# gaurav00700/Selfsupervised-NVSF

Hardware: AMD Instinct MI355X
Metric: rendered rays/sec (LiDAR+cam) (higher is better)
Workload: dtype f16; 1 GPU; C2: KITTI-360 seq-1908-shaped frame per GPU, uniform sampling, static hash field; num_rays=4096, num_rays_lidar=4096, num_steps=768, hash_grid=L16 F2 T2^19 base16 max2048, sigma_mlp=32-64-16, heads=lidar 2x(87-64-64-1), rgb 31-64-64-3, parallelism=frame-sharded x1, no collective

## Files before the change

selfsupervised-nvsf_amd/csrc/common.h:

```cpp
#pragma once
#include <hip/hip_runtime.h>
#include <stdint.h>

#define NVSF_API extern "C" __attribute__((visibility("default")))

enum : int {
    NVSF_OK = 0,
    NVSF_ERR_INVALID_ARG = -1,
    NVSF_ERR_UNSUPPORTED = -2,
};

constexpr int kWave = 64;

static inline int nvsf_launch_status() {
    hipError_t e = hipGetLastError();
    return e == hipSuccess ? NVSF_OK : (int)e;
}

static inline unsigned cdiv(unsigned long long a, unsigned b) { return (unsigned)((a + b - 1) / b); }

enum NvsfVariantKey : int {
    kVarMarch = 0,
    kVarPlanesFwd,
    kVarPlanesBwd,
    kVarHashgridFwd,
    kVarHashgridBwd,
    kVarHash4dBwd,
    kVarSlicePlan,
    kVarRenderTail,
    kVarMarchSkew,
    kVarMlpBwd,
    kVarLevelKinds,
    kVarCount
};
int nvsf_variant(int key);
int nvsf_cu_count();

__device__ __forceinline__ int lane_id() { return (int)(threadIdx.x & 63); }

template <typename T>
__device__ __forceinline__ T wave_sum(T v) {
#pragma unroll
    for (int o = 32; o > 0; o >>= 1) v += __shfl_xor(v, o, 64);
    return v;
}

__device__ __forceinline__ float wave_scan_add(float v) {
    const int l = lane_id();
#pragma unroll
    for (int o = 1; o < 64; o <<= 1) {
        float u = __shfl_up(v, o, 64);
        if (l >= o) v += u;
    }
    return v;
}
__device__ __forceinline__ float wave_scan_mul(float v) {
    const int l = lane_id();
#pragma unroll
    for (int o = 1; o < 64; o <<= 1) {
        float u = __shfl_up(v, o, 64);
        if (l >= o) v *= u;
    }
    return v;
}
__device__ __forceinline__ uint32_t wave_scan_add_u32(uint32_t v) {
    const int l = lane_id();
#pragma unroll
    for (int o = 1; o < 64; o <<= 1) {
        uint32_t u = __shfl_up(v, o, 64);
        if (l >= o) v += u;
    }
    return v;
}

__device__ __forceinline__ uint32_t wave_scan_max_u32(uint32_t v) {
#define NVSF_DPP_MAX(ctrl, row_mask)                                                                                        \
    {                                                                                                                      \
        const uint32_t u = (uint32_t)__builtin_amdgcn_update_dpp(0, (int)v, ctrl, row_mask, 0xF, false);                   \
        v = u > v ? u : v;                                                                                                 \
    }
    NVSF_DPP_MAX(0x111, 0xF)
    NVSF_DPP_MAX(0x112, 0xF)
    NVSF_DPP_MAX(0x114, 0xF)
    NVSF_DPP_MAX(0x118, 0xF)
    NVSF_DPP_MAX(0x142, 0xA)
    NVSF_DPP_MAX(0x143, 0xC)
#undef NVSF_DPP_MAX
    return v;
}
```

selfsupervised-nvsf_amd/csrc/fused_field.hip:

```cpp
#include "hashgrid_device.h"
#include "mlp_device.h"
#include "encodings_device.h"
#include "march_device.h"
#pragma clang diagnostic ignored "-Wpass-failed"
#include <stdlib.h>

namespace {
constexpr int kBlock = 256;
constexpr int kWavesPerBlock = kBlock / kWave;

struct RayBatch {
    const float* rays_o;
    const float* rays_d;
    const float* nears;
    const float* fars;
    const float* lin;
    const float* noise;
    float lo[3], hi[3];
    float inv_extent;
    float bound;
    uint32_t N, T;
};

template <int F>
// ... 18 lines not shown
        const unsigned long long s = in_range ? s_raw : total - 1;
        const uint32_t n = (uint32_t)(s / rb.T), i = (uint32_t)(s - (unsigned long long)n * rb.T);
        const float near = rb.nears[n], range = rb.fars[n] - near;
        float z = near + range * rb.lin[i];
        if (rb.noise) z = z + (rb.noise[s] - 0.5f) * (range / (float)rb.T);
        float x[3];
#pragma unroll
        for (int k = 0; k < 3; ++k) {
            float p = rb.rays_o[3 * (size_t)n + k] + rb.rays_d[3 * (size_t)n + k] * z;
            p = fminf(fmaxf(p, rb.lo[k]), rb.hi[k]);
            x[k] = (p + rb.bound) * rb.inv_extent;
        }
        half8_t xf;
#pragma unroll
        for (int q = 0; q < kLevelsPerGroup; ++q) {
            const int l = g * kLevelsPerGroup + q;
            float acc[F];
            encode_level<3, F>(x, table, meta.scale[l], meta.res[l], meta.offset[l], meta.offset[l + 1] - meta.offset[l], acc);
#pragma unroll
            for (int f = 0; f < F; ++f) xf[q * F + f] = (_Float16)acc[f];
        }
        float4_t acc1[kHidTiles];
#pragma unroll
        for (int t = 0; t < kHidTiles; ++t) {
            const float4_t zero = {0, 0, 0, 0};
            acc1[t] = mfma16(w0[t], xf, zero);
        }
        half8_t h[kHidSteps];
        pack_hidden(acc1, h);
        const float4_t o = wout.apply(h);
        if (in_range) {
            half4_t ov;
            ov[0] = (_Float16)o[0]; ov[1] = (_Float16)o[1]; ov[2] = (_Float16)o[2]; ov[3] = (_Float16)o[3];
            if (g == 3) {
                z_vals[s] = z;
                sigmas[s] = expf(o[3]);
                ov[3] = (_Float16)1.0f;
            }
            *reinterpret_cast<half4_t*>(geo + s * 16 + 4 * g) = ov;
        }
    }
}

template <int F>
struct LaneLevels {
    static constexpr int Q = 8 / F;
    float scale[Q];
    uint32_t res[Q], res2[Q], boff[Q], rows[Q];
};

__device__ __forceinline__ void fma_entry(float w, uint32_t raw, float& a0, float& a1) {
    asm("v_fma_mix_f32 %0, %1, %2, %0 op_sel_hi:[0,1,0]" : "+v"(a0) : "v"(w), "v"(raw));
    asm("v_fma_mix_f32 %0, %1, %2, %0 op_sel:[0,1,0] op_sel_hi:[0,1,0]" : "+v"(a1) : "v"(w), "v"(raw));
}

template <int F>
__device__ __forceinline__ uint32_t gather_raw(__amdgpu_buffer_rsrc_t rsrc, uint32_t byte_off);
template <>
__device__ __forceinline__ uint32_t gather_raw<2>(__amdgpu_buffer_rsrc_t rsrc, uint32_t byte_off) {
    return __builtin_amdgcn_raw_buffer_load_b32(rsrc, byte_off, 0, 0);
}
typedef uint32_t entry4_t __attribute__((ext_vector_type(2)));
template <int F> struct EntryOf { typedef uint32_t type; };
template <> struct EntryOf<4> { typedef entry4_t type; };
template <>
__device__ __forceinline__ uint32_t gather_raw<4>(__amdgpu_buffer_rsrc_t, uint32_t) = delete;
__device__ __forceinline__ entry4_t gather_raw4(__amdgpu_buffer_rsrc_t rsrc, uint32_t byte_off) {
    return __builtin_amdgcn_raw_buffer_load_b64(rsrc, byte_off, 0, 0);
}

template <int F>
struct DensityCtx {
    static constexpr int Q = 8 / F;
    LaneLevels<F> lv;
    half8_t w0[kHidTiles];
    OutLayerW wout;
    __amdgpu_buffer_rsrc_t rsrc;
    uint32_t first_hashed;
    int g;
    const uint4* lds_lv;
};

constexpr uint32_t kFirstHashedC2 = 5;
template <int F, int QG, bool LDS_LV = false, int FH = -1>
__device__ __forceinline__ half8_t density_encode(const DensityCtx<F>& cx, const float (&x)[3]) {
    constexpr int Q = 8 / F;
    LaneLevels<F> lv_local;
    if constexpr (LDS_LV) {
        uint32_t again = 0;
        asm volatile("" : "+v"(again));
#pragma unroll
        for (int q = 0; q < Q; ++q) {
            const uint4 v = cx.lds_lv[4 * q + again];
            lv_local.scale[q] = __builtin_bit_cast(float, v.x);
            lv_local.res[q] = v.y;
            lv_local.res2[q] = v.y * v.y;
            lv_local.boff[q] = v.z;
            lv_local.rows[q] = v.w;
        }
    }
    const LaneLevels<F>& lv = LDS_LV ? lv_local : cx.lv;
    const uint32_t first_hashed = FH >= 0 ? (uint32_t)FH : cx.first_hashed;
    const int g = cx.g;
    half8_t xf;
#pragma unroll
    for (int q0 = 0; q0 < Q; q0 += QG) {
    float frac[Q][3];
    typename EntryOf<F>::type raw[Q][8];
#pragma unroll
    for (int q = q0; q < q0 + QG; ++q) {
        uint32_t c[3];
#pragma unroll
        for (int d = 0; d < 3; ++d) {
            const float pos = fmaf(lv.scale[q], x[d], 0.5f);
            const float fl = floorf(pos);
            frac[q][d] = pos - fl;
            c[d] = (uint32_t)(int32_t)fl;
        }
        uint32_t idx[8];
        const bool all_dense = (uint32_t)(4 * q + 3) < first_hashed, all_hashed = (uint32_t)(4 * q) >= first_hashed;
        if (all_dense || !all_hashed) {
            const uint32_t b00 = c[0] + c[1] * lv.res[q] + c[2] * lv.res2[q];
            const uint32_t b10 = b00 + lv.res[q], b01 = b00 + lv.res2[q], b11 = b10 + lv.res2[q];
            const uint32_t base[4] = {b00, b10, b01, b11};
#pragma unroll
            for (int k = 0; k < 8; ++k) {
                uint32_t v = base[k >> 1] + (uint32_t)(k & 1);
                v = v >= lv.rows[q] ? v - lv.rows[q] : v;
                idx[k] = v;
            }
        }
        if (all_hashed || !all_dense) {
            const uint32_t hy0 = c[1] * 2654435761u, hy1 = hy0 + 2654435761u;
            const uint32_t hz0 = c[2] * 805459861u, hz1 = hz0 + 805459861u;
            const uint32_t yz[4] = {hy0 ^ hz0, hy1 ^ hz0, hy0 ^ hz1, hy1 ^ hz1};
            const uint32_t mask = lv.rows[q] - 1u;
            const bool lane_hashed = (uint32_t)(4 * q + g) >= first_hashed;
#pragma unroll
            for (int k = 0; k < 8; ++k) {
                const uint32_t v = ((c[0] + (uint32_t)(k & 1)) ^ yz[k >> 1]) & mask;
                idx[k] = (all_hashed || lane_hashed) ? v : idx[k];
            }
        }
#pragma unroll
        for (int k = 0; k < 8; ++k) {
            if constexpr (F == 2) raw[q][k] = gather_raw<2>(cx.rsrc, lv.boff[q] + idx[k] * (uint32_t)(F * sizeof(_Float16)));
            else raw[q][k] = gather_raw4(cx.rsrc, lv.boff[q] + idx[k] * (uint32_t)(F * sizeof(_Float16)));
        }
    }
#pragma unroll
    for (int q = q0; q < q0 + QG; ++q) {
        const float fx = frac[q][0], fy = frac[q][1], fz = frac[q][2];
        const float wx[2] = {1.0f - fx, fx}, wy[2] = {1.0f - fy, fy}, wz[2] = {1.0f - fz, fz};
        if constexpr (F == 2) {
            float a0 = 0.0f, a1 = 0.0f;
#pragma unroll
            for (int k = 0; k < 8; ++k) {
                const float w = (wx[k & 1] * wy[(k >> 1) & 1]) * wz[k >> 2];
                fma_entry(w, raw[q][k], a0, a1);
            }
            xf[q * F] = (_Float16)a0;
            xf[q * F + 1] = (_Float16)a1;
        } else {
            float a0 = 0.0f, a1 = 0.0f, a2 = 0.0f, a3 = 0.0f;
#pragma unroll
            for (int k = 0; k < 8; ++k) {
                const float w = (wx[k & 1] * wy[(k >> 1) & 1]) * wz[k >> 2];
                fma_entry(w, raw[q][k][0], a0, a1);
                fma_entry(w, raw[q][k][1], a2, a3);
            }
            xf[q * F] = (_Float16)a0;
            xf[q * F + 1] = (_Float16)a1;
            xf[q * F + 2] = (_Float16)a2;
            xf[q * F + 3] = (_Float16)a3;
        }
    }
    }
    return xf;
}

template <int F, int QG>
__device__ __forceinline__ float4_t density_eval(const DensityCtx<F>& cx, const float (&x)[3]) {
    const half8_t xf = density_encode<F, QG>(cx, x);
    float4_t acc1[kHidTiles];
#pragma unroll
    for (int t = 0; t < kHidTiles; ++t) {
        const float4_t zero = {0, 0, 0, 0};
        acc1[t] = mfma16(cx.w0[t], xf, zero);
    }
    half8_t h[kHidSteps];
    pack_hidden(acc1, h);
    return cx.wout.apply(h);
}

struct TrainOut {
    float* x01;
    _Float16* feat;
    float* h32;
    uint32_t* tile;
};

__device__ __forceinline__ void store_h32(float* __restrict__ h32, unsigned long long s, int lane, int g, float o0, float o1, float o2, float o3, bool ok) {
    const int from = (lane + 48) & 63;
    const float prev = __int_as_float(__builtin_amdgcn_ds_bpermute(from << 2, __float_as_int(o3)));
    if (ok) *reinterpret_cast<float4*>(h32 + s * 16 + 4 * g) = make_float4(prev, o0, o1, o2);
}

constexpr int kTrPitch = 20;
constexpr int kTrWords = 16 * kTrPitch;
__device__ __forceinline__ void store_feat_row(_Float16* __restrict__ feat, unsigned long long s, int lane, int g, const uint4& p, bool ok,
                                               uint32_t* tile) {
    uint32_t* row = tile + (lane & 15) * kTrPitch;
    row[g] = p.x; row[4 + g] = p.y; row[8 + g] = p.z; row[12 + g] = p.w;
    const uint4 mine = *reinterpret_cast<const uint4*>(row + 4 * g);
    if (ok) *reinterpret_cast<uint4*>(feat + s * 32 + 8 * g) = mine;
}

__device__ __forceinline__ void store_feat_row_swap(_Float16* __restrict__ feat, unsigned long long s, int g, const uint4& p, bool ok) {
    const auto a = __builtin_amdgcn_permlane16_swap(p.x, p.y, false, false);
    const auto b = __builtin_amdgcn_permlane16_swap(p.z, p.w, false, false);
    const auto lo = __builtin_amdgcn_permlane32_swap(a[0], b[0], false, false);
    const auto hi = __builtin_amdgcn_permlane32_swap(a[1], b[1], false, false);
    if (ok) *reinterpret_cast<uint4*>(feat + s * 32 + 8 * g) = make_uint4(lo[0], hi[0], lo[1], hi[1]);
}

template <int F, int QG, bool TRAIN = false>
__device__ __forceinline__ void density_tile(const DensityCtx<F>& cx, const float (&x)[3], float z, unsigned long long s, bool in_range,
                                             float* __restrict__ z_vals, float* __restrict__ sigmas, _Float16* __restrict__ geo,
                                             const TrainOut* tr = nullptr) {
    const int g = cx.g;
    float4_t o;
    if constexpr (TRAIN) {
        const half8_t xf = density_encode<F, QG>(cx, x);
        float4_t acc1[kHidTiles];
#pragma unroll
        for (int t = 0; t < kHidTiles; ++t) {
            const float4_t zero = {0, 0, 0, 0};
            acc1[t] = mfma16(cx.w0[t], xf, zero);
        }
        half8_t h[kHidSteps];
        pack_hidden(acc1, h);
        o = cx.wout.apply(h);
        const int lane = lane_id();
        store_feat_row(tr->feat, s, lane, g, __builtin_bit_cast(uint4, xf), in_range, tr->tile);
        store_h32(tr->h32, s, lane, g, o[0], o[1], o[2], o[3], in_range);
        if (in_range && g == 0) { tr->x01[3 * s] = x[0]; tr->x01[3 * s + 1] = x[1]; tr->x01[3 * s + 2] = x[2]; }
    } else {
        o = density_eval<F, QG>(cx, x);
    }
    if (in_range) {
        half4_t ov;
        ov[0] = (_Float16)o[0]; ov[1] = (_Float16)o[1]; ov[2] = (_Float16)o[2]; ov[3] = (_Float16)o[3];
        if (g == 3) {
            z_vals[s] = z;
            sigmas[s] = expf(o[3]);
            ov[3] = (_Float16)1.0f;
        }
        *reinterpret_cast<half4_t*>(geo + s * 16 + 4 * g) = ov;
    }
// ... 917 lines not shown
        }
        const float sigma = expf(o[3]) * density_scale;
        const uint32_t p0 = pack_h2(o[0], o[1]), p1 = pack_h2(o[2], g == 3 ? 1.0f : o[3]);
        typedef uint32_t u4_t __attribute__((ext_vector_type(4)));
        u4_t gv;
        gv[0] = (uint32_t)__shfl((int)p0, src_a);
        gv[1] = (uint32_t)__shfl((int)p1, src_a);
        gv[2] = (uint32_t)__shfl((int)p0, src_b);
        gv[3] = (uint32_t)__shfl((int)p1, src_b);
        const half8_t x_last = takes_geo ? __builtin_bit_cast(half8_t, gv) : xf[IN_STEPS - 1];
        float c[3] = {0.0f, 0.0f, 0.0f};
        const float4_t oa = head(0, x_last);
        if constexpr (LIDAR) {
            const float4_t ob = head(1, x_last);
            c[0] = sigmoid_f32(oa[0]);
            c[1] = sigmoid_f32(ob[0]);
        } else {
            c[0] = sigmoid_f32(oa[0]); c[1] = sigmoid_f32(oa[1]); c[2] = sigmoid_f32(oa[2]);
        }
#pragma unroll
        for (int i = 0; i < 16; ++i) {
            if ((uint32_t)i < cnt && alive) {
                const float s_i = readlane_f32(sigma, 48 + i);
                const float dt_i = readlane_f32(sdt, i), d1_i = readlane_f32(sd1, i);
                const float alpha = 1.0f - expf(-s_i * dt_i);
                const float T = 1.0f - ws;
                const float w = alpha * T;
                ws += w;
                t_comp += d1_i;
                dep += w * t_comp;
#pragma unroll
                for (int k = 0; k < 3; ++k) col[k] += w * readlane_f32(c[k], i);
                if (T < T_thresh) alive = false;
            }
        }
        total += cnt;
        if (cnt < 16u) alive = false;
    }
    if (lane == 0) {
        weights_sum[n] = ws;
        depth[n] = dep;
        if constexpr (LIDAR) {
            image[2 * (size_t)n] = col[0];
            image[2 * (size_t)n + 1] = col[1];
        } else {
            const float rest = 1.0f - ws;
            image[3 * (size_t)n] = col[0] + rest * bg0;
            image[3 * (size_t)n + 1] = col[1] + rest * bg1;
            image[3 * (size_t)n + 2] = col[2] + rest * bg2;
        }
    }
}

template <int N>
__device__ __forceinline__ float row_shr(float old, float v) {
    static_assert(N >= 1 && N <= 15, "row_shr:1..15");
    return __builtin_bit_cast(float, __builtin_amdgcn_update_dpp(__builtin_bit_cast(int, old), __builtin_bit_cast(int, v), 0x110 + N, 0xF, 0xF, false));
}

__device__ __forceinline__ float row_shl1(float old, float v) {
    return __builtin_bit_cast(float, __builtin_amdgcn_update_dpp(__builtin_bit_cast(int, old), __builtin_bit_cast(int, v), 0x101, 0xF, 0xF, false));
}

__device__ __forceinline__ float row_first(float v) {
    return __builtin_bit_cast(float, __builtin_amdgcn_update_dpp(0, __builtin_bit_cast(int, v), 0x150, 0xF, 0xF, false));
}

__device__ __forceinline__ float row16_scan_mul(float v) {
    v *= row_shr<1>(1.0f, v);
    v *= row_shr<2>(1.0f, v);
    v *= row_shr<4>(1.0f, v);
    v *= row_shr<8>(1.0f, v);
    return v;
}

struct RenderTrainOut {
    float* x01;
    _Float16* feat;
    _Float16* geo;
    float* sigma;
    float* rgb;
};

template <bool LIDAR, bool FROM_FEATURES, bool TRAIN = false, int FH = -1>
__global__ __launch_bounds__(kBlock) __attribute__((amdgpu_waves_per_eu(4, 4))) void k_render_uniform(
    RayBatch rb, const _Float16* __restrict__ table, uint32_t table_bytes, GridMeta meta, uint32_t first_hashed,
    const uint2* __restrict__ feat, const _Float16* __restrict__ w_sigma, const _Float16* __restrict__ w_a, const _Float16* __restrict__ w_b,
    float k_scale, float w_thresh, float bg0, float bg1, float bg2, int use_bg, float* __restrict__ z_vals, float* __restrict__ weights,
    float* __restrict__ weights_sum, float* __restrict__ depth, float* __restrict__ image, RenderTrainOut rt = RenderTrainOut()) {
    using FR = OccFrags<LIDAR>;
    constexpr int F = 2;
    constexpr int IN_STEPS = FR::IN_STEPS;
    constexpr int C = LIDAR ? 2 : 3;
    __shared__ uint4 s_lv[kMaxLevels];
    __shared__ half8_t s_frag[FR::kCount * kWave];
    __shared__ float4_t s_pre[kWavesPerBlock * FR::kPre];
    if (threadIdx.x < kMaxLevels) {
        const uint32_t l = threadIdx.x;
        s_lv[l] = make_uint4(__builtin_bit_cast(uint32_t, meta.scale[l]), meta.res[l], meta.offset[l] * (uint32_t)(F * sizeof(_Float16)),
                             meta.offset[l + 1] - meta.offset[l]);
    }
    const int lane = lane_id(), g = lane >> 4, c = lane & 15;
    for (int f = (int)(threadIdx.x >> 6); f < FR::kCount; f += kWavesPerBlock) s_frag[f * kWave + lane] = occ_fragment<LIDAR>(f, lane, w_sigma, w_a, w_b);
    __syncthreads();
    const uint32_t n = __builtin_amdgcn_readfirstlane(blockIdx.x * kWavesPerBlock + (threadIdx.x >> 6));
    if (n >= rb.N) return;
    const half8_t* frag = s_frag + lane;
    const uint32_t T = rb.T;
    const size_t M = (size_t)rb.N * T;

    DensityCtx<F> cx;
    if constexpr (!FROM_FEATURES) {
        cx.g = g;
        cx.first_hashed = first_hashed;
        cx.lds_lv = s_lv + g;
        cx.rsrc = __builtin_amdgcn_make_buffer_rsrc(const_cast<_Float16*>(table), 0, (int)table_bytes, 0x00020000);
    }
    const float rd0 = rb.rays_d[3 * (size_t)n], rd1 = rb.rays_d[3 * (size_t)n + 1], rd2 = rb.rays_d[3 * (size_t)n + 2];
    const float d0 = (rd0 + 1.0f) / 2.0f, d1 = (rd1 + 1.0f) / 2.0f, d2 = (rd2 + 1.0f) / 2.0f;
    half8_t xf[IN_STEPS];
    if constexpr (!LIDAR) {
        float sh[16];
        sh4_basis(d0, d1, d2, sh);
#pragma unroll
        for (int j = 0; j < 8; ++j) xf[0][j] = (_Float16)(g == 0 ? sh[j] : sh[8 + j]);
    } else {
#pragma unroll
        for (int s = 0; s < 3; ++s)
#pragma unroll
            for (int j = 0; j < 8; j += 2) {
                const int k = 32 * s + 8 * g + j;
                float sn = 1.0f, cs = 1.0f;
                if (k < 72) {
                    const int i = k / 24, f = (k - 24 * i) >> 1;
                    freq_pair(i == 0 ? d0 : (i == 1 ? d1 : d2), f, sn, cs);
                }
                xf[s][j] = (_Float16)sn;
                xf[s][j + 1] = (_Float16)cs;
            }
    }
    const bool takes_geo = LIDAR ? (g == 1 || g == 2) : (g >= 2);
    const int src_a = (c + 16 * (LIDAR ? 2 * (g - 1) : 2 * (g - 2))) & 63, src_b = (src_a + 16) & 63;
    float4_t* pre = s_pre + (threadIdx.x >> 6) * FR::kPre;
    ray_head_constants<LIDAR>(xf, w_a, w_b, lane, pre);
    auto head = [&](int hd, const half8_t& x_last) {
        const int base = FR::kHead + hd * FR::kPerHead;
        float4_t acc[kHidTiles];
#pragma unroll
        for (int t = 0; t < kHidTiles; ++t) {
            float4_t c = {0, 0, 0, 0};
            if constexpr (IN_STEPS > 1) c = pre[(hd * 4 + t) * 4 + g];
            acc[t] = mfma16(frag[(base + t) * kWave], x_last, c);
        }
        half8_t h[kHidSteps];
        pack_hidden(acc, h);
#pragma unroll
        for (int t = 0; t < kHidTiles; ++t) {
            float4_t c = {0, 0, 0, 0};
#pragma unroll
            for (int s = 0; s < kHidSteps; ++s) c = mfma16(frag[(base + 4 + 2 * t + s) * kWave], h[s], c);
            acc[t] = c;
        }
        pack_hidden(acc, h);
        float4_t c = {0, 0, 0, 0};
#pragma unroll
        for (int s = 0; s < kHidSteps; ++s) c = mfma16(frag[(base + 4 + 8 + s) * kWave], h[s], c);
        return c;
    };

    const float near = rb.nears[n], range = rb.fars[n] - near;
    const float sample_dist = range / (float)T;
    const float ox = rb.rays_o[3 * (size_t)n], oy = rb.rays_o[3 * (size_t)n + 1], oz = rb.rays_o[3 * (size_t)n + 2];
    const size_t row0 = (size_t)n * T;
    float carry = 1.0f, ws = 0.0f, dp = 0.0f, img[C];
#pragma unroll
    for (int k = 0; k < C; ++k) img[k] = 0.0f;
    float lin_cur = 0.0f, lin_nxt = 0.0f, nz_cur = 0.5f, nz_nxt = 0.5f;
    auto request = [&](uint32_t i0) {
        const uint32_t i = i0 + (uint32_t)c;
        const uint32_t ic = i < T ? i : T - 1u, in = ic + 1u < T ? ic + 1u : ic;
        lin_cur = rb.lin[ic];
        lin_nxt = rb.lin[in];
        if (rb.noise) {
            nz_cur = rb.noise[row0 + ic];
            nz_nxt = rb.noise[row0 + in];
        }
    };
    if constexpr (!FROM_FEATURES) request(0u);
    for (uint32_t i0 = 0; i0 < T; i0 += 16) {
        const uint32_t i = i0 + (uint32_t)c;
        const bool valid = i < T;
        const uint32_t ic = valid ? i : T - 1u;
        const size_t s = row0 + ic;
        float z, z_next;
        half8_t feat8;
        if constexpr (FROM_FEATURES) {
            z = z_vals[s];
            z_next = ic + 1u < T ? z_vals[s + 1] : z;
            const uint2 p0 = feat[(size_t)(2 * g) * M + s], p1 = feat[(size_t)(2 * g + 1) * M + s];
            typedef uint32_t u4_t __attribute__((ext_vector_type(4)));
            const u4_t packed = {p0.x, p1.x, p1.y, p0.y};
            feat8 = __builtin_bit_cast(half8_t, packed);
        } else {
            z = near + range * lin_cur;
            z_next = near + range * lin_nxt;
            if (rb.noise) {
                z = z + (nz_cur - 0.5f) * sample_dist;
                z_next = z_next + (nz_nxt - 0.5f) * sample_dist;
            }
            if (i0 + 16u < T) request(i0 + 16u);
            float x[3];
            x[0] = (fminf(fmaxf(ox + rd0 * z, rb.lo[0]), rb.hi[0]) + rb.bound) * rb.inv_extent;
            x[1] = (fminf(fmaxf(oy + rd1 * z, rb.lo[1]), rb.hi[1]) + rb.bound) * rb.inv_extent;
            x[2] = (fminf(fmaxf(oz + rd2 * z, rb.lo[2]), rb.hi[2]) + rb.bound) * rb.inv_extent;
            feat8 = density_encode<F, 4, true, FH>(cx, x);
            if constexpr (TRAIN) {
                if (g == 0 && valid) { rt.x01[3 * s] = x[0]; rt.x01[3 * s + 1] = x[1]; rt.x01[3 * s + 2] = x[2]; }
            }
        }
        if constexpr (TRAIN) store_feat_row_swap(rt.feat, s, g, __builtin_bit_cast(uint4, feat8), valid);
        float4_t o;
        {
            float4_t acc1[kHidTiles];
#pragma unroll
            for (int tt = 0; tt < kHidTiles; ++tt) acc1[tt] = mfma16(frag[(FR::kSigma + tt) * kWave], feat8, float4_t{0, 0, 0, 0});
            half8_t h[kHidSteps];
            pack_hidden(acc1, h);
            float4_t a = {0, 0, 0, 0};
#pragma unroll
            for (int sx = 0; sx < kHidSteps; ++sx) a = mfma16(frag[(FR::kSigma + 4 + sx) * kWave], h[sx], a);
            o = a;
        }
        const float delta = (i + 1u < T) ? z_next - z : sample_dist;
        float alpha = 0.0f;
        if (g == 3 && valid) alpha = 1.0f - expf(-delta * k_scale * expf(o[3]));
        const float om = (g == 3 && valid) ? (1.0f - alpha + 1e-15f) : 1.0f;
        const float incl = row16_scan_mul(om);
        const float excl = row_shr<1>(1.0f, incl);
        const float w = alpha * (carry * excl);
        carry = carry * readlane_f32(incl, 63);
        if (g == 3 && valid) {
            weights[s] = w;
            if constexpr (!FROM_FEATURES) z_vals[s] = z;
            if constexpr (TRAIN) rt.sigma[s] = expf(o[3]);
        }
        ws += w;
        dp += w * z;
        const float w0 = __shfl(w, 48 + c, 64);
        const bool on = w0 > w_thresh;
        float cr[C];
#pragma unroll
        for (int k = 0; k < C; ++k) cr[k] = 0.0f;
        if constexpr (TRAIN) {
            if (valid) *reinterpret_cast<uint2*>(rt.geo + s * 16 + 4 * g) = make_uint2(pack_h2(o[0], o[1]), pack_h2(o[2], g == 3 ? 1.0f : o[3]));
        }
        if (__ballot(w > w_thresh)) {
            const uint32_t p0 = pack_h2(o[0], o[1]), p1 = pack_h2(o[2], g == 3 ? 1.0f : o[3]);
            typedef uint32_t u4_t __attribute__((ext_vector_type(4)));
            u4_t gv;
            gv[0] = (uint32_t)__shfl((int)p0, src_a);
            gv[1] = (uint32_t)__shfl((int)p1, src_a);
            gv[2] = (uint32_t)__shfl((int)p0, src_b);
            gv[3] = (uint32_t)__shfl((int)p1, src_b);
            const half8_t x_last = takes_geo ? __builtin_bit_cast(half8_t, gv) : xf[IN_STEPS - 1];
            const float4_t oa = head(0, x_last);
            if constexpr (LIDAR) {
                const float4_t ob = head(1, x_last);
                if (g == 0 && on) {
                    cr[0] = sigmoid_f32(oa[0]);
                    cr[1] = sigmoid_f32(ob[0]);
                    img[0] += w0 * cr[0];
                    img[1] += w0 * cr[1];
                }
            } else {
                if (g == 0 && on) {
#pragma unroll
                    for (int k = 0; k < 3; ++k) {
                        cr[k] = sigmoid_f32(oa[k]);
                        img[k] += w0 * cr[k];
                    }
                }
            }
        }
        if constexpr (TRAIN) {
            if (g == 0 && valid) {
#pragma unroll
                for (int k = 0; k < C; ++k) rt.rgb[s * C + k] = cr[k];
            }
        }
    }
    ws = wave_sum(ws);
    dp = wave_sum(dp);
#pragma unroll
    for (int k = 0; k < C; ++k) img[k] = wave_sum(img[k]);
    if (lane == 0) {
        weights_sum[n] = ws;
        depth[n] = dp;
// ... 459 lines not shown
    REQUIRE(rays_o && rays_d && nears && fars && grid && table_f16 && sigma_weights_f16 && head_a_weights_f16 && weights_sum && depth && image);
    REQUIRE(!lidar || head_b_weights_f16);
    REQUIRE(bound > 0.0f && C >= 1 && C <= 8 && H >= 2 && H <= 1024 && max_steps >= 1);
    REQUIRE((reinterpret_cast<uintptr_t>(table_f16) & 15u) == 0 && (reinterpret_cast<uintptr_t>(sigma_weights_f16) & 15u) == 0 &&
            (reinterpret_cast<uintptr_t>(head_a_weights_f16) & 15u) == 0 && (reinterpret_cast<uintptr_t>(head_b_weights_f16) & 15u) == 0);
    if ((F != 2 && F != 4) || L * F != 32) return NVSF_ERR_UNSUPPORTED;
    GridMeta meta;
    const int st = fill_meta(meta, L, h_scales, h_res, h_offsets);
    if (st != NVSF_OK) return st;
    uint32_t first_hashed = L;
    for (uint32_t l = 0; l < L; ++l) {
        const unsigned long long cells = (unsigned long long)h_res[l] * h_res[l] * h_res[l];
        const uint32_t rows = h_offsets[l + 1] - h_offsets[l];
        const bool hashed = cells > (unsigned long long)rows;
        if (hashed && first_hashed == L) first_hashed = l;
        if (!hashed && first_hashed != L) return NVSF_ERR_UNSUPPORTED;
        if (hashed && (rows & (rows - 1u)) != 0u) return NVSF_ERR_UNSUPPORTED;
    }
    const unsigned long long table_bytes = (unsigned long long)h_offsets[L] * F * sizeof(_Float16);
    if (table_bytes >= (1ull << 31)) return NVSF_ERR_UNSUPPORTED;
    OccRays rr;
    rr.rays_o = rays_o; rr.rays_d = rays_d; rr.nears = nears; rr.fars = fars; rr.grid = grid;
    rr.bound = bound; rr.dt_gamma = dt_gamma; rr.max_steps = max_steps; rr.C = C; rr.H = H; rr.N = N;
    const _Float16* tb = reinterpret_cast<const _Float16*>(table_f16);
    const _Float16* ws = reinterpret_cast<const _Float16*>(sigma_weights_f16);
    const _Float16* wa = reinterpret_cast<const _Float16*>(head_a_weights_f16);
    const _Float16* wb = reinterpret_cast<const _Float16*>(head_b_weights_f16);
    const float b0 = h_bg_color ? h_bg_color[0] : 0.0f, b1 = h_bg_color ? h_bg_color[1] : 0.0f, b2 = h_bg_color ? h_bg_color[2] : 0.0f;
    const dim3 grid_dim(cdiv(N, kWavesPerBlock)), block(kBlock);
#define LAUNCH_OCC(LD, FF, FH)                                                                                                            \
    hipLaunchKernelGGL((k_render_occupancy_lds<LD, FF, FH>), grid_dim, block, 0, stream, rr, tb, (uint32_t)table_bytes, meta, first_hashed, ws, \
                       wa, wb, density_scale, T_thresh, b0, b1, b2, weights_sum, depth, image)
    const bool c2_grid = F == 2 && first_hashed == kFirstHashedC2 && nvsf_variant(kVarLevelKinds) == 0;
    if (lidar) { if (c2_grid) LAUNCH_OCC(true, 2, (int)kFirstHashedC2); else if (F == 2) LAUNCH_OCC(true, 2, -1); else LAUNCH_OCC(true, 4, -1); }
    else { if (c2_grid) LAUNCH_OCC(false, 2, (int)kFirstHashedC2); else if (F == 2) LAUNCH_OCC(false, 2, -1); else LAUNCH_OCC(false, 4, -1); }
#undef LAUNCH_OCC
    return nvsf_launch_status();
}

static int render_uniform_impl(const float* rays_o, const float* rays_d, const float* nears, const float* fars, const float* lin,
                               const float* noise, const float* h_aabb, float bound, uint32_t N, uint32_t T, const void* table_f16,
                               uint32_t L, uint32_t F, const float* h_scales, const uint32_t* h_res, const uint32_t* h_offsets,
                               const void* sigma_weights_f16, int lidar, const void* head_a_weights_f16,
                               const void* head_b_weights_f16, float k_scale, float w_thresh, const float* h_bg_color,
                               const void* feat_scratch, float* z_vals, float* weights, float* weights_sum, float* depth, float* image,
                               hipStream_t stream, const RenderTrainOut* train) {
    if (N == 0 || T == 0) return NVSF_OK;
    REQUIRE(rays_o && rays_d && nears && fars && h_aabb && table_f16 && sigma_weights_f16 && head_a_weights_f16);
    REQUIRE(z_vals && weights && weights_sum && depth && image && (feat_scratch || lin));
    REQUIRE(!lidar || head_b_weights_f16);
    REQUIRE(bound > 0.0f);
    REQUIRE((reinterpret_cast<uintptr_t>(table_f16) & 15u) == 0 && (reinterpret_cast<uintptr_t>(sigma_weights_f16) & 15u) == 0 &&
            (reinterpret_cast<uintptr_t>(head_a_weights_f16) & 15u) == 0 && (reinterpret_cast<uintptr_t>(head_b_weights_f16) & 15u) == 0 &&
            (reinterpret_cast<uintptr_t>(feat_scratch) & 15u) == 0);
    if (!((F == 2 && L == 16) || (F == 4 && L == 8 && feat_scratch))) return NVSF_ERR_UNSUPPORTED;
    GridMeta meta;
    const int st = fill_meta(meta, L, h_scales, h_res, h_offsets);
    if (st != NVSF_OK) return st;
    uint32_t first_hashed = L;
    for (uint32_t l = 0; l < L; ++l) {
        const unsigned long long cells = (unsigned long long)h_res[l] * h_res[l] * h_res[l];
        const uint32_t rows = h_offsets[l + 1] - h_offsets[l];
        const bool hashed = cells > (unsigned long long)rows;
        if (hashed && first_hashed == L) first_hashed = l;
        if (!hashed && first_hashed != L) return NVSF_ERR_UNSUPPORTED;
        if (hashed && (rows & (rows - 1u)) != 0u) return NVSF_ERR_UNSUPPORTED;
    }
    const unsigned long long table_bytes = (unsigned long long)h_offsets[L] * F * sizeof(_Float16);
    if (table_bytes >= (1ull << 31)) return NVSF_ERR_UNSUPPORTED;
    RayBatch rb;
    rb.rays_o = rays_o; rb.rays_d = rays_d; rb.nears = nears; rb.fars = fars; rb.lin = lin; rb.noise = noise;
    for (int k = 0; k < 3; ++k) { rb.lo[k] = h_aabb[k]; rb.hi[k] = h_aabb[3 + k]; }
    rb.bound = bound;
    rb.inv_extent = 1.0f / (2.0f * bound);
    rb.N = N; rb.T = T;
    const _Float16* tb = reinterpret_cast<const _Float16*>(table_f16);
    const _Float16* ws = reinterpret_cast<const _Float16*>(sigma_weights_f16);
    const _Float16* wa = reinterpret_cast<const _Float16*>(head_a_weights_f16);
    const _Float16* wb = reinterpret_cast<const _Float16*>(head_b_weights_f16);
    const uint2* fp = reinterpret_cast<const uint2*>(feat_scratch);
    const float b0 = h_bg_color ? h_bg_color[0] : 0.0f, b1 = h_bg_color ? h_bg_color[1] : 0.0f, b2 = h_bg_color ? h_bg_color[2] : 0.0f;
    const int use_bg = (h_bg_color && !lidar) ? 1 : 0;
    const dim3 grid_dim(cdiv(N, kWavesPerBlock)), block(kBlock);
#define LAUNCH_RU_FH(LD, FF, FH)                                                                                                      \
    do {                                                                                                                              \
        if (train)                                                                                                                    \
            hipLaunchKernelGGL((k_render_uniform<LD, FF, true, FH>), grid_dim, block, 0, stream, rb, tb, (uint32_t)table_bytes, meta, \
                               first_hashed, fp, ws, wa, wb, k_scale, w_thresh, b0, b1, b2, use_bg, z_vals, weights, weights_sum,     \
                               depth, image, *train);                                                                                \
        else                                                                                                                          \
            hipLaunchKernelGGL((k_render_uniform<LD, FF, false, FH>), grid_dim, block, 0, stream, rb, tb, (uint32_t)table_bytes,      \
                               meta, first_hashed, fp, ws, wa, wb, k_scale, w_thresh, b0, b1, b2, use_bg, z_vals, weights,            \
                               weights_sum, depth, image, RenderTrainOut());                                                         \
    } while (0)
#define LAUNCH_RU(LD, FF)                                                                                                             \
    do {                                                                                                                              \
        if (!FF && first_hashed == kFirstHashedC2 && nvsf_variant(kVarLevelKinds) == 0) LAUNCH_RU_FH(LD, FF, (FF ? -1 : (int)kFirstHashedC2)); \
        else LAUNCH_RU_FH(LD, FF, -1);                                                                                                \
    } while (0)
#define LAUNCH_TAIL(LD)                                                                                                               \
    do {                                                                                                                              \
        if (train)                                                                                                                    \
            hipLaunchKernelGGL((k_render_tail2<LD, true>), grid_dim, block, 0, stream, rb, fp, ws, wa, wb, k_scale, w_thresh, b0, b1, \
                               b2, use_bg, z_vals, weights, weights_sum, depth, image, *train);                                      \
        else                                                                                                                          \
            hipLaunchKernelGGL((k_render_tail2<LD, false>), grid_dim, block, 0, stream, rb, fp, ws, wa, wb, k_scale, w_thresh, b0,    \
                               b1, b2, use_bg, z_vals, weights, weights_sum, depth, image, RenderTrainOut());                        \
    } while (0)
    const bool tail2 = nvsf_variant(kVarRenderTail) == 0;
    if (lidar) { if (fp) { if (tail2) LAUNCH_TAIL(true); else LAUNCH_RU(true, true); } else LAUNCH_RU(true, false); }
    else { if (fp) { if (tail2) LAUNCH_TAIL(false); else LAUNCH_RU(false, true); } else LAUNCH_RU(false, false); }
#undef LAUNCH_TAIL
#undef LAUNCH_RU
#undef LAUNCH_RU_FH
    return nvsf_launch_status();
}

NVSF_API int nvsf_render_uniform_fwd(const float* rays_o, const float* rays_d, const float* nears, const float* fars, const float* lin,
                                     const float* noise, const float* h_aabb, float bound, uint32_t N, uint32_t T, const void* table_f16,
                                     uint32_t L, uint32_t F, const float* h_scales, const uint32_t* h_res, const uint32_t* h_offsets,
                                     const void* sigma_weights_f16, int lidar, const void* head_a_weights_f16,
                                     const void* head_b_weights_f16, float k_scale, float w_thresh, const float* h_bg_color,
                                     const void* feat_scratch, float* z_vals, float* weights, float* weights_sum, float* depth, float* image,
                                     hipStream_t stream) {
    return render_uniform_impl(rays_o, rays_d, nears, fars, lin, noise, h_aabb, bound, N, T, table_f16, L, F, h_scales, h_res, h_offsets,
                               sigma_weights_f16, lidar, head_a_weights_f16, head_b_weights_f16, k_scale, w_thresh, h_bg_color, feat_scratch,
                               z_vals, weights, weights_sum, depth, image, stream, nullptr);
}

NVSF_API int nvsf_render_uniform_train_fwd(const float* rays_o, const float* rays_d, const float* nears, const float* fars, const float* lin,
                                           const float* noise, const float* h_aabb, float bound, uint32_t N, uint32_t T,
                                           const void* table_f16, uint32_t L, uint32_t F, const float* h_scales, const uint32_t* h_res,
                                           const uint32_t* h_offsets, const void* sigma_weights_f16, int lidar,
                                           const void* head_a_weights_f16, const void* head_b_weights_f16, float k_scale, float w_thresh,
                                           const float* h_bg_color, void* feat_scratch, float* z_vals, float* weights, float* weights_sum,
                                           float* depth, float* image, float* x01, void* feat_rows_f16, void* geo_f16, float* sigmas,
                                           float* rgbs, hipStream_t stream) {
    if (N == 0 || T == 0) return NVSF_OK;
    REQUIRE(x01 && feat_rows_f16 && geo_f16 && sigmas && rgbs && lin);
    REQUIRE((reinterpret_cast<uintptr_t>(feat_rows_f16) & 15u) == 0 && (reinterpret_cast<uintptr_t>(geo_f16) & 15u) == 0);
    RenderTrainOut rt;
    rt.x01 = x01; rt.feat = reinterpret_cast<_Float16*>(feat_rows_f16); rt.geo = reinterpret_cast<_Float16*>(geo_f16);
    rt.sigma = sigmas; rt.rgb = rgbs;
    if (feat_scratch) {
        TrainOut tr;
        tr.x01 = x01; tr.feat = rt.feat; tr.h32 = nullptr; tr.tile = nullptr;
        const int st = density_uniform_impl(rays_o, rays_d, nears, fars, lin, noise, h_aabb, bound, N, T, table_f16, L, F, h_scales, h_res, h_offsets,
                                            sigma_weights_f16, z_vals, sigmas, geo_f16, feat_scratch, 1u, stream, &tr);
        if (st != NVSF_OK) return st;
    }
    return render_uniform_impl(rays_o, rays_d, nears, fars, lin, noise, h_aabb, bound, N, T, table_f16, L, F, h_scales, h_res, h_offsets,
                               sigma_weights_f16, lidar, head_a_weights_f16, head_b_weights_f16, k_scale, w_thresh, h_bg_color, feat_scratch,
                               z_vals, weights, weights_sum, depth, image, stream, &rt);
}
```

selfsupervised-nvsf_amd/csrc/version.hip:

```cpp
#include "common.h"
#include <string.h>
NVSF_API const char* nvsf_version(void) { return "nvsf_hip 0.1.0 gfx950"; }

#ifndef NVSF_CSRC_DIGEST_ALL
#define NVSF_CSRC_DIGEST_ALL "unknown_________"
#endif
#ifndef NVSF_CSRC_DIGEST_RENDER
#define NVSF_CSRC_DIGEST_RENDER "unknown_________"
#endif
#define NVSF_MARK_ALL "NVSF_CSRC_DIGEST_ALL="
#define NVSF_MARK_RENDER "NVSF_CSRC_DIGEST_RENDER="
static const char g_digest_all[] = NVSF_MARK_ALL NVSF_CSRC_DIGEST_ALL;
static const char g_digest_render[] = NVSF_MARK_RENDER NVSF_CSRC_DIGEST_RENDER;
NVSF_API const char* nvsf_build_digest(int which) {
    return which == 1 ? g_digest_render + sizeof(NVSF_MARK_RENDER) - 1 : g_digest_all + sizeof(NVSF_MARK_ALL) - 1;
}

static int g_variant[kVarCount] = {};
__attribute__((visibility("hidden"))) int nvsf_variant(int key) { return key >= 0 && key < kVarCount ? g_variant[key] : 0; }

__attribute__((visibility("hidden"))) int nvsf_cu_count() {
    static const int n = [] {
        int dev = 0, v = 0;
        if (hipGetDevice(&dev) != hipSuccess || hipDeviceGetAttribute(&v, hipDeviceAttributeMultiprocessorCount, dev) != hipSuccess || v <= 0) v = 256;
        return v;
    }();
    return n;
}

NVSF_API int nvsf_test_variant(const char* name, int value) {
    static const char* const names[kVarCount] = {"march", "planes_fwd", "planes_bwd", "hashgrid_fwd", "hashgrid_bwd", "hash4d_bwd", "slice_plan",
                                                 "render_tail", "march_skew", "mlp_bwd", "level_kinds"};
    if (!name || value < 0) return NVSF_ERR_INVALID_ARG;
    for (int k = 0; k < kVarCount; ++k)
        if (strcmp(name, names[k]) == 0) {
            const int old = g_variant[k];
            g_variant[k] = value;
            return old;
        }
    return NVSF_ERR_INVALID_ARG;
}
```

selfsupervised-nvsf_amd/nvsf/testing.py:

```python
import contextlib

_NATIVE = {
    "march": {"wave": 0, "thread": 1, "serial": 2},
    "planes_fwd": {"runs": 0, "sample": 1},
    "planes_bwd": {"runs": 0, "atomic": 1, "global": 2},
    "hashgrid_fwd": {"auto": 0, "generic": 1},
    "hashgrid_bwd": {"corners": 0, "atomic": 1},
    "hash4d_bwd": {"lds": 0, "runs": 1},
    "slice_plan": {"balanced": 0, "home": 1},
    "render_tail": {"two": 0, "one": 1},
    "mlp_bwd": {"auto": 0, "staged": 1, "wave": 2},
    "level_kinds": {"compiled": 0, "runtime": 1},
    "march_skew": {"off": 0, **{f"queue{q}": q + 1 for q in range(8)}},
}
_PYTHON = {
    "heads_input": ("prefix", "rows"),
    "density_sliced": (None, False, True),
    "hash4d_train": ("fused", "slices"),
    "dynamic_fused": (True, False),
    "density_tail_train": ("fused", "chain"),
    "density_fn": ("fused", "chain"),
    "planes_train": ("fused", "separate"),
    "density_grad": ("composed", "matrix"),
    "hash4d_scatter": ("side", "main"),
    "table_scatter": ("binned", "atomic"),
}
_state = {}


def get(name):
    return _state.get(name, _PYTHON[name][0])


@contextlib.contextmanager
def variant(**choices):
    from nvsf import _hip
    lib = _hip.load()
    undo_native, undo_python = [], []
    try:
        for name, value in choices.items():
            if name in _NATIVE:
                code = _NATIVE[name][value]
                old = lib.nvsf_test_variant(name.encode(), code)
                if old < 0:
                    raise _hip.NvsfHipError(f"nvsf_test_variant({name!r}) rejected")
                undo_native.append((name, old))
            elif name in _PYTHON:
                if value not in _PYTHON[name]:
                    raise ValueError(f"{name}: one of {_PYTHON[name]}")
                undo_python.append((name, _state.get(name, _PYTHON[name][0])))
                _state[name] = value
            else:
                raise KeyError(name)
        yield
    finally:
        for name, old in reversed(undo_native):
            lib.nvsf_test_variant(name.encode(), old)
        for name, old in reversed(undo_python):
            _state[name] = old
```

Measured before the change: 12.80 million rays/s.

## Prefetch last hash-grid level gathers one sample tile ahead in uniform render

Splits density encoding into separate issue and blend steps so the uniform render kernel can issue the hash-table gathers for the last level group of the next 16-sample tile before it blends the current one. This aims to hide gather latency behind the MLP and compositing work of the current tile. The cost is extra live registers for the in-flight gathers, which could spill or lower occupancy given the fixed waves-per-EU setting. It is on by default through a new variant switch.

```diff
diff --git a/selfsupervised-nvsf_amd/csrc/common.h b/selfsupervised-nvsf_amd/csrc/common.h
--- a/selfsupervised-nvsf_amd/csrc/common.h
+++ b/selfsupervised-nvsf_amd/csrc/common.h
@@ -31,6 +31,7 @@
     kVarMarchSkew,
     kVarMlpBwd,
     kVarLevelKinds,
+    kVarRenderPrefetch,
     kVarCount
 };
 int nvsf_variant(int key);
diff --git a/selfsupervised-nvsf_amd/csrc/fused_field.hip b/selfsupervised-nvsf_amd/csrc/fused_field.hip
--- a/selfsupervised-nvsf_amd/csrc/fused_field.hip
+++ b/selfsupervised-nvsf_amd/csrc/fused_field.hip
@@ -124,99 +124,114 @@
 };
 
 constexpr uint32_t kFirstHashedC2 = 5;
+template <int F>
+struct LevelGathers {
+    float frac[3];
+    typename EntryOf<F>::type raw[8];
+};
+
+template <int F>
+__device__ __forceinline__ void lane_levels_lds(const DensityCtx<F>& cx, LaneLevels<F>& lv) {
+    constexpr int Q = 8 / F;
+    uint32_t again = 0;
+    asm volatile("" : "+v"(again));
+#pragma unroll
+    for (int q = 0; q < Q; ++q) {
+        const uint4 v = cx.lds_lv[4 * q + again];
+        lv.scale[q] = __builtin_bit_cast(float, v.x);
+        lv.res[q] = v.y;
+        lv.res2[q] = v.y * v.y;
+        lv.boff[q] = v.z;
+        lv.rows[q] = v.w;
+    }
+}
+
+template <int F, int FH>
+__device__ __forceinline__ void level_issue(const DensityCtx<F>& cx, const LaneLevels<F>& lv, int q, const float (&x)[3], LevelGathers<F>& lg) {
+    const uint32_t first_hashed = FH >= 0 ? (uint32_t)FH : cx.first_hashed;
+    const int g = cx.g;
+    uint32_t c[3];
+#pragma unroll
+    for (int d = 0; d < 3; ++d) {
+        const float pos = fmaf(lv.scale[q], x[d], 0.5f);
+        const float fl = floorf(pos);
+        lg.frac[d] = pos - fl;
+        c[d] = (uint32_t)(int32_t)fl;
+    }
+    uint32_t idx[8];
+    const bool all_dense = (uint32_t)(4 * q + 3) < first_hashed, all_hashed = (uint32_t)(4 * q) >= first_hashed;
+    if (all_dense || !all_hashed) {
+        const uint32_t b00 = c[0] + c[1] * lv.res[q] + c[2] * lv.res2[q];
+        const uint32_t b10 = b00 + lv.res[q], b01 = b00 + lv.res2[q], b11 = b10 + lv.res2[q];
+        const uint32_t base[4] = {b00, b10, b01, b11};
+#pragma unroll
+        for (int k = 0; k < 8; ++k) {
+            uint32_t v = base[k >> 1] + (uint32_t)(k & 1);
+            v = v >= lv.rows[q] ? v - lv.rows[q] : v;
+            idx[k] = v;
+        }
+    }
+    if (all_hashed || !all_dense) {
+        const uint32_t hy0 = c[1] * 2654435761u, hy1 = hy0 + 2654435761u;
+        const uint32_t hz0 = c[2] * 805459861u, hz1 = hz0 + 805459861u;
+        const uint32_t yz[4] = {hy0 ^ hz0, hy1 ^ hz0, hy0 ^ hz1, hy1 ^ hz1};
+        const uint32_t mask = lv.rows[q] - 1u;
+        const bool lane_hashed = (uint32_t)(4 * q + g) >= first_hashed;
+#pragma unroll
+        for (int k = 0; k < 8; ++k) {
+            const uint32_t v = ((c[0] + (uint32_t)(k & 1)) ^ yz[k >> 1]) & mask;
+            idx[k] = (all_hashed || lane_hashed) ? v : idx[k];
+        }
+    }
+#pragma unroll
+    for (int k = 0; k < 8; ++k) {
+        if constexpr (F == 2) lg.raw[k] = gather_raw<2>(cx.rsrc, lv.boff[q] + idx[k] * (uint32_t)(F * sizeof(_Float16)));
+        else lg.raw[k] = gather_raw4(cx.rsrc, lv.boff[q] + idx[k] * (uint32_t)(F * sizeof(_Float16)));
+    }
+}
+
+template <int F>
+__device__ __forceinline__ void level_blend(const LevelGathers<F>& lg, int q, half8_t& xf) {
+    const float fx = lg.frac[0], fy = lg.frac[1], fz = lg.frac[2];
+    const float wx[2] = {1.0f - fx, fx}, wy[2] = {1.0f - fy, fy}, wz[2] = {1.0f - fz, fz};
+    if constexpr (F == 2) {
+        float a0 = 0.0f, a1 = 0.0f;
+#pragma unroll
+        for (int k = 0; k < 8; ++k) {
+            const float w = (wx[k & 1] * wy[(k >> 1) & 1]) * wz[k >> 2];
+            fma_entry(w, lg.raw[k], a0, a1);
+        }
+        xf[q * F] = (_Float16)a0;
+        xf[q * F + 1] = (_Float16)a1;
+    } else {
+        float a0 = 0.0f, a1 = 0.0f, a2 = 0.0f, a3 = 0.0f;
+#pragma unroll
+        for (int k = 0; k < 8; ++k) {
+            const float w = (wx[k & 1] * wy[(k >> 1) & 1]) * wz[k >> 2];
+            fma_entry(w, lg.raw[k][0], a0, a1);
+            fma_entry(w, lg.raw[k][1], a2, a3);
+        }
+        xf[q * F] = (_Float16)a0;
+        xf[q * F + 1] = (_Float16)a1;
+        xf[q * F + 2] = (_Float16)a2;
+        xf[q * F + 3] = (_Float16)a3;
+    }
+}
+
 template <int F, int QG, bool LDS_LV = false, int FH = -1>
 __device__ __forceinline__ half8_t density_encode(const DensityCtx<F>& cx, const float (&x)[3]) {
     constexpr int Q = 8 / F;
     LaneLevels<F> lv_local;
-    if constexpr (LDS_LV) {
-        uint32_t again = 0;
-        asm volatile("" : "+v"(again));
-#pragma unroll
-        for (int q = 0; q < Q; ++q) {
-            const uint4 v = cx.lds_lv[4 * q + again];
-            lv_local.scale[q] = __builtin_bit_cast(float, v.x);
-            lv_local.res[q] = v.y;
-            lv_local.res2[q] = v.y * v.y;
-            lv_local.boff[q] = v.z;
-            lv_local.rows[q] = v.w;
-        }
-    }
+    if constexpr (LDS_LV) lane_levels_lds(cx, lv_local);
     const LaneLevels<F>& lv = LDS_LV ? lv_local : cx.lv;
-    const uint32_t first_hashed = FH >= 0 ? (uint32_t)FH : cx.first_hashed;
-    const int g = cx.g;
     half8_t xf;
 #pragma unroll
     for (int q0 = 0; q0 < Q; q0 += QG) {
-    float frac[Q][3];
-    typename EntryOf<F>::type raw[Q][8];
-#pragma unroll
-    for (int q = q0; q < q0 + QG; ++q) {
-        uint32_t c[3];
-#pragma unroll
-        for (int d = 0; d < 3; ++d) {
-            const float pos = fmaf(lv.scale[q], x[d], 0.5f);
-            const float fl = floorf(pos);
-            frac[q][d] = pos - fl;
-            c[d] = (uint32_t)(int32_t)fl;
-        }
-        uint32_t idx[8];
-        const bool all_dense = (uint32_t)(4 * q + 3) < first_hashed, all_hashed = (uint32_t)(4 * q) >= first_hashed;
-        if (all_dense || !all_hashed) {
-            const uint32_t b00 = c[0] + c[1] * lv.res[q] + c[2] * lv.res2[q];
-            const uint32_t b10 = b00 + lv.res[q], b01 = b00 + lv.res2[q], b11 = b10 + lv.res2[q];
-            const uint32_t base[4] = {b00, b10, b01, b11};
-#pragma unroll
-            for (int k = 0; k < 8; ++k) {
-                uint32_t v = base[k >> 1] + (uint32_t)(k & 1);
-                v = v >= lv.rows[q] ? v - lv.rows[q] : v;
-                idx[k] = v;
-            }
-        }
-        if (all_hashed || !all_dense) {
-            const uint32_t hy0 = c[1] * 2654435761u, hy1 = hy0 + 2654435761u;
-            const uint32_t hz0 = c[2] * 805459861u, hz1 = hz0 + 805459861u;
-            const uint32_t yz[4] = {hy0 ^ hz0, hy1 ^ hz0, hy0 ^ hz1, hy1 ^ hz1};
-            const uint32_t mask = lv.rows[q] - 1u;
-            const bool lane_hashed = (uint32_t)(4 * q + g) >= first_hashed;
-#pragma unroll
-            for (int k = 0; k < 8; ++k) {
-                const uint32_t v = ((c[0] + (uint32_t)(k & 1)) ^ yz[k >> 1]) & mask;
-                idx[k] = (all_hashed || lane_hashed) ? v : idx[k];
-            }
-        }
-#pragma unroll
-        for (int k = 0; k < 8; ++k) {
-            if constexpr (F == 2) raw[q][k] = gather_raw<2>(cx.rsrc, lv.boff[q] + idx[k] * (uint32_t)(F * sizeof(_Float16)));
-            else raw[q][k] = gather_raw4(cx.rsrc, lv.boff[q] + idx[k] * (uint32_t)(F * sizeof(_Float16)));
-        }
-    }
-#pragma unroll
-    for (int q = q0; q < q0 + QG; ++q) {
-        const float fx = frac[q][0], fy = frac[q][1], fz = frac[q][2];
-        const float wx[2] = {1.0f - fx, fx}, wy[2] = {1.0f - fy, fy}, wz[2] = {1.0f - fz, fz};
-        if constexpr (F == 2) {
-            float a0 = 0.0f, a1 = 0.0f;
-#pragma unroll
-            for (int k = 0; k < 8; ++k) {
-                const float w = (wx[k & 1] * wy[(k >> 1) & 1]) * wz[k >> 2];
-                fma_entry(w, raw[q][k], a0, a1);
-            }
-            xf[q * F] = (_Float16)a0;
-            xf[q * F + 1] = (_Float16)a1;
-        } else {
-            float a0 = 0.0f, a1 = 0.0f, a2 = 0.0f, a3 = 0.0f;
-#pragma unroll
-            for (int k = 0; k < 8; ++k) {
-                const float w = (wx[k & 1] * wy[(k >> 1) & 1]) * wz[k >> 2];
-                fma_entry(w, raw[q][k][0], a0, a1);
-                fma_entry(w, raw[q][k][1], a2, a3);
-            }
-            xf[q * F] = (_Float16)a0;
-            xf[q * F + 1] = (_Float16)a1;
-            xf[q * F + 2] = (_Float16)a2;
-            xf[q * F + 3] = (_Float16)a3;
-        }
-    }
+        LevelGathers<F> lg[QG];
+#pragma unroll
+        for (int q = q0; q < q0 + QG; ++q) level_issue<F, FH>(cx, lv, q, x, lg[q - q0]);
+#pragma unroll
+        for (int q = q0; q < q0 + QG; ++q) level_blend(lg[q - q0], q, xf);
     }
     return xf;
 }
@@ -1300,12 +1315,15 @@
     float* rgb;
 };
 
-template <bool LIDAR, bool FROM_FEATURES, bool TRAIN = false, int FH = -1>
+constexpr int kRenderAhead = 1;
+constexpr int kRenderAheadTrain = 1;
+template <bool LIDAR, bool FROM_FEATURES, bool TRAIN = false, int FH = -1, int AHEAD = 0>
 __global__ __launch_bounds__(kBlock) __attribute__((amdgpu_waves_per_eu(4, 4))) void k_render_uniform(
     RayBatch rb, const _Float16* __restrict__ table, uint32_t table_bytes, GridMeta meta, uint32_t first_hashed,
     const uint2* __restrict__ feat, const _Float16* __restrict__ w_sigma, const _Float16* __restrict__ w_a, const _Float16* __restrict__ w_b,
     float k_scale, float w_thresh, float bg0, float bg1, float bg2, int use_bg, float* __restrict__ z_vals, float* __restrict__ weights,
     float* __restrict__ weights_sum, float* __restrict__ depth, float* __restrict__ image, RenderTrainOut rt = RenderTrainOut()) {
+    static_assert(AHEAD >= 0 && AHEAD < 4 && (AHEAD == 0 || !FROM_FEATURES), "AHEAD: level steps of the gathering form issued a tile ahead");
     using FR = OccFrags<LIDAR>;
     constexpr int F = 2;
     constexpr int IN_STEPS = FR::IN_STEPS;
@@ -1404,7 +1422,32 @@
             nz_nxt = rb.noise[row0 + in];
         }
     };
+    auto sample_z = [&](float& z, float& z_next) {
+        z = near + range * lin_cur;
+        z_next = near + range * lin_nxt;
+        if (rb.noise) {
+            z = z + (nz_cur - 0.5f) * sample_dist;
+            z_next = z_next + (nz_nxt - 0.5f) * sample_dist;
+        }
+    };
+    auto unit_point = [&](float z, float (&x)[3]) {
+        x[0] = (fminf(fmaxf(ox + rd0 * z, rb.lo[0]), rb.hi[0]) + rb.bound) * rb.inv_extent;
+        x[1] = (fminf(fmaxf(oy + rd1 * z, rb.lo[1]), rb.hi[1]) + rb.bound) * rb.inv_extent;
+        x[2] = (fminf(fmaxf(oz + rd2 * z, rb.lo[2]), rb.hi[2]) + rb.bound) * rb.inv_extent;
+    };
+    constexpr int QA = 4 - AHEAD;
+    float z_a = 0.0f, zn_a = 0.0f, x_a[3] = {0.0f, 0.0f, 0.0f};
+    LevelGathers<F> ahead[AHEAD > 0 ? AHEAD : 1];
+    auto issue_ahead = [&]() {
+        sample_z(z_a, zn_a);
+        unit_point(z_a, x_a);
+        LaneLevels<F> lv;
+        lane_levels_lds(cx, lv);
+#pragma unroll
+        for (int q = QA; q < 4; ++q) level_issue<F, FH>(cx, lv, q, x_a, ahead[q - QA]);
+    };
     if constexpr (!FROM_FEATURES) request(0u);
+    if constexpr (AHEAD > 0) issue_ahead();
     for (uint32_t i0 = 0; i0 < T; i0 += 16) {
         const uint32_t i = i0 + (uint32_t)c;
         const bool valid = i < T;
@@ -1419,18 +1462,29 @@
             typedef uint32_t u4_t __attribute__((ext_vector_type(4)));
             const u4_t packed = {p0.x, p1.x, p1.y, p0.y};
             feat8 = __builtin_bit_cast(half8_t, packed);
+        } else if constexpr (AHEAD > 0) {
+            z = z_a;
+            z_next = zn_a;
+            const float x[3] = {x_a[0], x_a[1], x_a[2]};
+            request(i0 + 16u);
+            LaneLevels<F> lv;
+            lane_levels_lds(cx, lv);
+            LevelGathers<F> lg[QA];
+#pragma unroll
+            for (int q = 0; q < QA; ++q) level_issue<F, FH>(cx, lv, q, x, lg[q]);
+#pragma unroll
+            for (int q = 0; q < QA; ++q) level_blend(lg[q], q, feat8);
+#pragma unroll
+            for (int q = QA; q < 4; ++q) level_blend(ahead[q - QA], q, feat8);
+            issue_ahead();
+            if constexpr (TRAIN) {
+                if (g == 0 && valid) { rt.x01[3 * s] = x[0]; rt.x01[3 * s + 1] = x[1]; rt.x01[3 * s + 2] = x[2]; }
+            }
         } else {
-            z = near + range * lin_cur;
-            z_next = near + range * lin_nxt;
-            if (rb.noise) {
-                z = z + (nz_cur - 0.5f) * sample_dist;
-                z_next = z_next + (nz_nxt - 0.5f) * sample_dist;
-            }
+            sample_z(z, z_next);
             if (i0 + 16u < T) request(i0 + 16u);
             float x[3];
-            x[0] = (fminf(fmaxf(ox + rd0 * z, rb.lo[0]), rb.hi[0]) + rb.bound) * rb.inv_extent;
-            x[1] = (fminf(fmaxf(oy + rd1 * z, rb.lo[1]), rb.hi[1]) + rb.bound) * rb.inv_extent;
-            x[2] = (fminf(fmaxf(oz + rd2 * z, rb.lo[2]), rb.hi[2]) + rb.bound) * rb.inv_extent;
+            unit_point(z, x);
             feat8 = density_encode<F, 4, true, FH>(cx, x);
             if constexpr (TRAIN) {
                 if (g == 0 && valid) { rt.x01[3 * s] = x[0]; rt.x01[3 * s + 1] = x[1]; rt.x01[3 * s + 2] = x[2]; }
@@ -2056,16 +2110,22 @@
     const float b0 = h_bg_color ? h_bg_color[0] : 0.0f, b1 = h_bg_color ? h_bg_color[1] : 0.0f, b2 = h_bg_color ? h_bg_color[2] : 0.0f;
     const int use_bg = (h_bg_color && !lidar) ? 1 : 0;
     const dim3 grid_dim(cdiv(N, kWavesPerBlock)), block(kBlock);
+    const bool ahead = nvsf_variant(kVarRenderPrefetch) == 0;
+#define LAUNCH_RU_K(LD, FF, FH, AH)                                                                                                   \
+    do {                                                                                                                              \
+        if (train)                                                                                                                    \
+            hipLaunchKernelGGL((k_render_uniform<LD, FF, true, FH, (FF || !AH) ? 0 : kRenderAheadTrain>), grid_dim, block, 0, stream, \
+                               rb, tb, (uint32_t)table_bytes, meta, first_hashed, fp, ws, wa, wb, k_scale, w_thresh, b0, b1, b2,      \
+                               use_bg, z_vals, weights, weights_sum, depth, image, *train);                                           \
+        else                                                                                                                          \
+            hipLaunchKernelGGL((k_render_uniform<LD, FF, false, FH, (FF || !AH) ? 0 : kRenderAhead>), grid_dim, block, 0, stream,     \
+                               rb, tb, (uint32_t)table_bytes, meta, first_hashed, fp, ws, wa, wb, k_scale, w_thresh, b0, b1, b2,      \
+                               use_bg, z_vals, weights, weights_sum, depth, image, RenderTrainOut());                                \
+    } while (0)
 #define LAUNCH_RU_FH(LD, FF, FH)                                                                                                      \
     do {                                                                                                                              \
-        if (train)                                                                                                                    \
-            hipLaunchKernelGGL((k_render_uniform<LD, FF, true, FH>), grid_dim, block, 0, stream, rb, tb, (uint32_t)table_bytes, meta, \
-                               first_hashed, fp, ws, wa, wb, k_scale, w_thresh, b0, b1, b2, use_bg, z_vals, weights, weights_sum,     \
-                               depth, image, *train);                                                                                \
-        else                                                                                                                          \
-            hipLaunchKernelGGL((k_render_uniform<LD, FF, false, FH>), grid_dim, block, 0, stream, rb, tb, (uint32_t)table_bytes,      \
-                               meta, first_hashed, fp, ws, wa, wb, k_scale, w_thresh, b0, b1, b2, use_bg, z_vals, weights,            \
-                               weights_sum, depth, image, RenderTrainOut());                                                         \
+        if (ahead) LAUNCH_RU_K(LD, FF, FH, 1);                                                                                        \
+        else LAUNCH_RU_K(LD, FF, FH, 0);                                                                                              \
     } while (0)
 #define LAUNCH_RU(LD, FF)                                                                                                             \
     do {                                                                                                                              \
@@ -2087,6 +2147,7 @@
 #undef LAUNCH_TAIL
 #undef LAUNCH_RU
 #undef LAUNCH_RU_FH
+#undef LAUNCH_RU_K
     return nvsf_launch_status();
 }
 
diff --git a/selfsupervised-nvsf_amd/csrc/version.hip b/selfsupervised-nvsf_amd/csrc/version.hip
--- a/selfsupervised-nvsf_amd/csrc/version.hip
+++ b/selfsupervised-nvsf_amd/csrc/version.hip
@@ -30,7 +30,7 @@
 
 NVSF_API int nvsf_test_variant(const char* name, int value) {
     static const char* const names[kVarCount] = {"march", "planes_fwd", "planes_bwd", "hashgrid_fwd", "hashgrid_bwd", "hash4d_bwd", "slice_plan",
-                                                 "render_tail", "march_skew", "mlp_bwd", "level_kinds"};
+                                                 "render_tail", "march_skew", "mlp_bwd", "level_kinds", "render_prefetch"};
     if (!name || value < 0) return NVSF_ERR_INVALID_ARG;
     for (int k = 0; k < kVarCount; ++k)
         if (strcmp(name, names[k]) == 0) {
diff --git a/selfsupervised-nvsf_amd/nvsf/testing.py b/selfsupervised-nvsf_amd/nvsf/testing.py
--- a/selfsupervised-nvsf_amd/nvsf/testing.py
+++ b/selfsupervised-nvsf_amd/nvsf/testing.py
@@ -11,6 +11,7 @@
     "render_tail": {"two": 0, "one": 1},
     "mlp_bwd": {"auto": 0, "staged": 1, "wave": 2},
     "level_kinds": {"compiled": 0, "runtime": 1},
+    "render_prefetch": {"ahead": 0, "off": 1},
     "march_skew": {"off": 0, **{f"queue{q}": q + 1 for q in range(8)}},
 }
 _PYTHON = {
```

Result: no change. 12.75 million rays/s (median of 2 runs) (-0.4%).
